# iacopoermacora/Street-sparse-3DGS

Measured on AMD Instinct MI355X. Metric: fwd+bwd Mpix/s at 1080p (1M Gaussians), higher is better.
Workload: dtype f32; 1 GPU; rasterizer fwd+bwd, 1000000 Gaussians, SH degree 3, 1920x1080, do_depth; gaussians=1000000, width=1920, height=1080, sh_degree=3, tiles=8160, fwd_segment=2048, parallelism=chunk-per-gpu x1

## Files before the change

### street-sparse-3dgs_amd/csrc/backward.hip

```cpp
#include <algorithm>
#include <atomic>

#include "gsr_launch.h"

namespace gsr {

#ifndef GSR_RED_SERIAL
#define GSR_RED_SERIAL 32
#endif
constexpr uint32_t kRedSerial = GSR_RED_SERIAL;
#ifndef GSR_REC_BATCH
#define GSR_REC_BATCH 4
#endif
#ifndef GSR_LIVE_UNROLL
#define GSR_LIVE_UNROLL 8
#endif
#ifndef GSR_BIG_BLOCK
#define GSR_BIG_BLOCK 2
#endif
constexpr int kRecBatch = GSR_REC_BATCH;

template <int D, bool kRow = false>
__device__ __forceinline__ void sh_backward(const float *__restrict__ sh, int M, bool vec, const float dir[3],
                                            const float gc[3], float *__restrict__ dsh, float gd[3]) {
// ... 188 lines not shown
            for (int j = 0; j < kBigBlock; j++) {
                q[0] += ra[j].x; q[1] += ra[j].y; q[2] += ra[j].z; q[3] += ra[j].w;
                q[4] += rb[j].x; q[5] += rb[j].y; q[6] += rb[j].z; q[7] += rb[j].w;
                q[8] += rc[j].x; q[9] += rc[j].y;
            }
        }
#pragma unroll
        for (int k = 0; k < 10; k++) {
            const float t = wave_sum(q[k]);
            if (lane == bl) g[k] = t;
        }
    }
    if (!valid) return;
    dmeans2D[3 * i + 0] = g[0];
    dmeans2D[3 * i + 1] = g[1];
    dmeans2D[3 * i + 2] = 0.f;
    dopacity[i] = g[5];
    sc.gsum[2 * (size_t)i] = make_float4(g[2], g[3], g[4], g[9]);
    sc.gsum[2 * (size_t)i + 1] = make_float4(g[6], g[7], g[8], 0.f);
}

constexpr int kShPitch = 13;
__device__ __forceinline__ void st_out(float *p, float v) { __builtin_nontemporal_store(v, p); }
__device__ __forceinline__ void st_out(float4 *p, float4 v) {
    typedef float f4 __attribute__((ext_vector_type(4)));
    __builtin_nontemporal_store(f4{v.x, v.y, v.z, v.w}, reinterpret_cast<f4 *>(p));
}

__device__ __forceinline__ void geom_chain(int i, float3 p, const Mat4 &V, const float *__restrict__ projmatrix, float fx,
                                           float fy, float tanx, float tany, bool has_scales,
                                           const float *__restrict__ scales, const float *__restrict__ rotations,
                                           float mod, const float *__restrict__ cov3D_precomp, const float g[10],
                                           float c3[6], float4 &q, float3 &s_in, float dm[3], float dcov[6],
                                           int raw) {
    if (has_scales) {
        s_in = make_float3(scales[3 * i], scales[3 * i + 1], scales[3 * i + 2]);
        q = reinterpret_cast<const float4 *>(rotations)[i];
        if (raw) {
            s_in = make_float3(act_scale(s_in.x), act_scale(s_in.y), act_scale(s_in.z));
            q = act_rot(q);
        }
        cov3d_from_scale_rot(s_in, mod, q, c3);
    } else {
#pragma unroll
        for (int k = 0; k < 6; k++) c3[k] = cov3D_precomp[6 * i + k];
    }
    const Ewa e = ewa_rows(p, V, fx, fy, tanx, tany);
    const float a = quad_form(e.m0, c3, e.m0) + 0.3f;
    const float b = quad_form(e.m0, c3, e.m1);
    const float c = quad_form(e.m1, c3, e.m1) + 0.3f;
    const float gca = g[2], gcb = g[3], gcc = g[4];
    const float denom = a * c - b * b;
    const float denom2inv = 1.0f / ((denom * denom) + 0.0000001f);
    float dL_da = 0.f, dL_db = 0.f, dL_dc = 0.f;
    if (denom2inv != 0.f) {
        dL_da = denom2inv * (-c * c * gca + 2.f * b * c * gcb + (denom - a * c) * gcc);
        dL_dc = denom2inv * (-a * a * gcc + 2.f * a * b * gcb + (denom - a * c) * gca);
        dL_db = denom2inv * 2.f * (b * c * gca - (denom + 2.f * b * b) * gcb + a * b * gcc);
        const float *m0 = e.m0, *m1 = e.m1;
        dcov[0] = m0[0] * m0[0] * dL_da + m0[0] * m1[0] * dL_db + m1[0] * m1[0] * dL_dc;
        dcov[3] = m0[1] * m0[1] * dL_da + m0[1] * m1[1] * dL_db + m1[1] * m1[1] * dL_dc;
        dcov[5] = m0[2] * m0[2] * dL_da + m0[2] * m1[2] * dL_db + m1[2] * m1[2] * dL_dc;
        dcov[1] = 2.f * m0[0] * m0[1] * dL_da + (m0[0] * m1[1] + m0[1] * m1[0]) * dL_db +
                  2.f * m1[0] * m1[1] * dL_dc;
        dcov[2] = 2.f * m0[0] * m0[2] * dL_da + (m0[0] * m1[2] + m0[2] * m1[0]) * dL_db +
                  2.f * m1[0] * m1[2] * dL_dc;
        dcov[4] = 2.f * m0[2] * m0[1] * dL_da + (m0[1] * m1[2] + m0[2] * m1[1]) * dL_db +
                  2.f * m1[1] * m1[2] * dL_dc;
    }
    float Sm0[3], Sm1[3];
    const float *m0 = e.m0, *m1 = e.m1;
    Sm0[0] = c3[0] * m0[0] + c3[1] * m0[1] + c3[2] * m0[2];
    Sm0[1] = c3[1] * m0[0] + c3[3] * m0[1] + c3[4] * m0[2];
    Sm0[2] = c3[2] * m0[0] + c3[4] * m0[1] + c3[5] * m0[2];
    Sm1[0] = c3[0] * m1[0] + c3[1] * m1[1] + c3[2] * m1[2];
    Sm1[1] = c3[1] * m1[0] + c3[3] * m1[1] + c3[4] * m1[2];
    Sm1[2] = c3[2] * m1[0] + c3[4] * m1[1] + c3[5] * m1[2];
    float dm0[3], dm1[3];
#pragma unroll
    for (int k = 0; k < 3; k++) {
        dm0[k] = 2.f * Sm0[k] * dL_da + Sm1[k] * dL_db;
        dm1[k] = 2.f * Sm1[k] * dL_dc + Sm0[k] * dL_db;
    }
    const float *v = V.m;
    const float dj00 = v[0] * dm0[0] + v[4] * dm0[1] + v[8] * dm0[2];
    const float dj02 = v[2] * dm0[0] + v[6] * dm0[1] + v[10] * dm0[2];
    const float dj11 = v[1] * dm1[0] + v[5] * dm1[1] + v[9] * dm1[2];
    const float dj12 = v[2] * dm1[0] + v[6] * dm1[1] + v[10] * dm1[2];
    const float tz = 1.f / e.t.z, tz2 = tz * tz, tz3 = tz2 * tz;
    const float dtx = e.xmul * -fx * tz2 * dj02;
    const float dty = e.ymul * -fy * tz2 * dj12;
    const float dtz = -fx * tz2 * dj00 - fy * tz2 * dj11 + (2.f * fx * e.t.x) * tz3 * dj02 +
                      (2.f * fy * e.t.y) * tz3 * dj12;
    dm[0] = v[0] * dtx + v[1] * dty + v[2] * dtz;
    dm[1] = v[4] * dtx + v[5] * dty + v[6] * dtz;
    dm[2] = v[8] * dtx + v[9] * dty + v[10] * dtz;

    const Mat4 Pm = load_mat4(projmatrix);
    const float *pr = Pm.m;
    const float4 mh = xf_point44(p, Pm);
    const float mw = 1.0f / (mh.w + 0.0000001f);
    const float mul1 = mh.x * mw * mw, mul2 = mh.y * mw * mw;
    dm[0] += (pr[0] * mw - pr[3] * mul1) * g[0] + (pr[1] * mw - pr[3] * mul2) * g[1];
    dm[1] += (pr[4] * mw - pr[7] * mul1) * g[0] + (pr[5] * mw - pr[7] * mul2) * g[1];
    dm[2] += (pr[8] * mw - pr[11] * mul1) * g[0] + (pr[9] * mw - pr[11] * mul2) * g[1];

    {
        const float3 pv = xf_point43(p, V);
        const float dz = -g[9] / (pv.z * pv.z);
        dm[0] += dz * v[2];
        dm[1] += dz * v[6];
        dm[2] += dz * v[10];
    }
}

__device__ __forceinline__ void scale_rot_chain(float4 q, float3 s_in, float mod, float dscale_mod, const float dcov[6],
                                                float ds[3], float dq[4]) {
    const float r = q.x, x = q.y, y = q.z, z = q.w;
    const float s[3] = {mod * s_in.x, mod * s_in.y, mod * s_in.z};
    const Rot3 R = quat_to_rot(q);
    const float G3[3][3] = {{dcov[0], 0.5f * dcov[1], 0.5f * dcov[2]},
                            {0.5f * dcov[1], dcov[3], 0.5f * dcov[4]},
                            {0.5f * dcov[2], 0.5f * dcov[4], dcov[5]}};
    float dLL[3][3];
#pragma unroll
    for (int rr = 0; rr < 3; rr++)
#pragma unroll
        for (int cc = 0; cc < 3; cc++)
            dLL[rr][cc] = 2.f * (G3[rr][0] * R.m[0][cc] * s[cc] + G3[rr][1] * R.m[1][cc] * s[cc] +
                                 G3[rr][2] * R.m[2][cc] * s[cc]);
#pragma unroll
// ... 280 lines not shown
        st_out(&out.dscales[3 * i + 0], 0.f);
        st_out(&out.dscales[3 * i + 1], 0.f);
        st_out(&out.dscales[3 * i + 2], 0.f);
    }
    if (valid && !live) st_out(&reinterpret_cast<float4 *>(out.drots)[i], z4);
    float4 *dst4 = reinterpret_cast<float4 *>(out.dsh) + row0 * 12;
#pragma unroll
    for (int k = 0; k < 12; k++) {
        const int f = k * kWave + lane, row = f / 12;
        if (row0 + row < P && !((lm >> row) & 1ull)) st_out(&dst4[f], z4);
    }
}

constexpr int kLiveRange = 2048;
constexpr int kLiveBlocksPerCU = 2;

struct LiveArgs {
    int P, D;
    const float *means3D, *shs;
    const uint8_t *clamped;
    const float *scales, *rotations;
    float mod, dscale_mod;
    const float *viewmatrix, *projmatrix, *campos;
    float tanx, tany, fx, fy;
    BwdScratch sc;
    GaussianGrads out;
    int raw, stamped;
    StepAct act;
};

__device__ __forceinline__ void live_row(int i, const Mat4 &V, int D, const float *__restrict__ means3D,
                                         const float *__restrict__ shs, const uint8_t *__restrict__ clamped,
                                         const float *__restrict__ scales, const float *__restrict__ rotations,
                                         float mod, float dscale_mod, const float *__restrict__ projmatrix,
                                         const float *__restrict__ campos_p, float tanx, float tany, float fx, float fy,
                                         const BwdScratch &sc, const GaussianGrads &out, int raw, int stamped,
                                         const StepAct &act) {
    float g[10];
    load_sums(sc, out, i, true, g);
    const float3 p = make_float3(means3D[3 * i], means3D[3 * i + 1], means3D[3 * i + 2]);
    float dm[3] = {0.f, 0.f, 0.f};
    float dcov[6] = {0.f, 0.f, 0.f, 0.f, 0.f, 0.f};
    float c3[6];
    float4 q = make_float4(0.f, 0.f, 0.f, 0.f);
    float3 s_in = make_float3(0.f, 0.f, 0.f);
    geom_chain(i, p, V, projmatrix, fx, fy, tanx, tany, true, scales, rotations, mod, nullptr, g, c3, q,
               s_in, dm, dcov, raw);
    if (stamped) {
        st_out(&out.dmeans2D[3 * i + 0], g[0]);
        st_out(&out.dmeans2D[3 * i + 1], g[1]);
        st_out(&out.dmeans2D[3 * i + 2], out.sparse_rows ? 1.f : 0.f);
        st_out(&out.dopacity[i], g[5]);
    }
    if (sc.atomic) {
        float4 *acc = sc.acc + 4 * (size_t)i;
        const float4 z4 = make_float4(0.f, 0.f, 0.f, 0.f);
#pragma unroll
        for (int k = 0; k < 4; k++) acc[k] = z4;
    }
    float dir[3], dor[3];
    sh_dir(p, make_float3(campos_p[0], campos_p[1], campos_p[2]), dir, dor);
    const uint8_t cl = clamped[i];
    float gc[3];
#pragma unroll
    for (int ch = 0; ch < 3; ch++) gc[ch] = (cl >> ch) & 1 ? 0.f : g[6 + ch];
    float gd[3];
    const float *sh = shs + (size_t)i * 48;
    float *dsh = out.dsh + (size_t)i * 48;
    switch (D) {
        case 0: sh_backward<0>(sh, 16, true, dir, gc, dsh, gd); break;
        case 1: sh_backward<1>(sh, 16, true, dir, gc, dsh, gd); break;
        case 2: sh_backward<2>(sh, 16, true, dir, gc, dsh, gd); break;
        default: sh_backward<3>(sh, 16, true, dir, gc, dsh, gd); break;
    }
    dir_chain(dor, gd, dm);
    st_out(&out.dmeans3D[3 * i + 0], dm[0]);
    st_out(&out.dmeans3D[3 * i + 1], dm[1]);
    st_out(&out.dmeans3D[3 * i + 2], dm[2]);
    float ds[3], dq[4];
    scale_rot_chain(q, s_in, mod, dscale_mod, dcov, ds, dq);
    if (act.on) {
#pragma unroll
        for (int k = 0; k < 3; k++) ds[k] = ds[k] * act_scale(act.s_raw[3 * i + k]);
        const float4 x = act.q_raw[i];
        const float4 gq = make_float4(dq[0], dq[1], dq[2], dq[3]);
        const float nq = sqrtf(x.x * x.x + x.y * x.y + x.z * x.z + x.w * x.w);
        const float d = fmaxf(nq, 1e-12f);
        const float gd =
            -(gq.x * ((x.x / d) / d) + gq.y * ((x.y / d) / d) + gq.z * ((x.z / d) / d) + gq.w * ((x.w / d) / d));
        const float gn = nq >= 1e-12f && nq != 0.f ? gd / nq : 0.f;
        dq[0] = gq.x / d + x.x * gn;
        dq[1] = gq.y / d + x.y * gn;
        dq[2] = gq.z / d + x.z * gn;
        dq[3] = gq.w / d + x.w * gn;
        const float y = act_opacity(act.o_raw[i]);
        const float go = (int64_t)i < act.skybox ? 0.f : g[5] * (1.f - y) * y;
        st_out(&out.dopacity[i], go);
        if (go != 0.f) *act.flag = 1;
        const int r = act.radii[i];
        if (r > 0) {
            const float gx = g[0], gy = g[1];
            const float nn = sqrtf(gx * gx + gy * gy);
            act.maxr[i] = fmaxf(act.maxr[i], (float)r);
            act.accum[i] = fmaxf(nn, act.accum[i]);
            act.denom[i] = act.denom[i] + 1.f;
        }
    }
    st_out(&out.dscales[3 * i + 0], ds[0]);
    st_out(&out.dscales[3 * i + 1], ds[1]);
    st_out(&out.dscales[3 * i + 2], ds[2]);
    st_out(&reinterpret_cast<float4 *>(out.drots)[i], make_float4(dq[0], dq[1], dq[2], dq[3]));
}

__device__ __forceinline__ void range_compact(const LiveArgs a, int64_t base, const uint32_t *__restrict__ stamps,
                                              uint32_t stamp, uint32_t *s_off, uint8_t *s_byte, uint64_t &m,
                                              uint32_t &byte) {
    const int t = threadIdx.x;
    const int P = a.P;
    const int nw = (P + 63) / 64;
    const int wi = (int)(base / 64) + t / 8;
    if (stamps) {
        byte = 0u;
        const int64_t r0 = base + 8 * t;
#pragma unroll
        for (int k = 0; k < 8; k++)
            if (r0 + k < P && stamps[r0 + k] == stamp) byte |= 1u << k;
        s_byte[t] = (uint8_t)byte;
        __syncthreads();
        m = 0ull;
#pragma unroll
        for (int k = 0; k < 8; k++) m |= (uint64_t)s_byte[(t & ~7) + k] << (8 * k);
    } else {
        m = wi < nw ? a.sc.live[wi] : 0ull;
        byte = (uint32_t)(m >> (8 * (t & 7))) & 0xFFu;
    }
    if ((t & 7) == 0) s_off[t / 8] = (uint32_t)__popcll(m);
    __syncthreads();
    if (t == 0) {
// ... 2 lines not shown
            const uint32_t c = s_off[k];
            s_off[k] = run;
            run += c;
        }
        s_off[kLiveRange / 64] = run;
    }
    __syncthreads();
}

__device__ __forceinline__ void nonlive_stats(const LiveArgs a, int64_t base, uint32_t byte) {
    if (!a.act.on) return;
    const int64_t r0 = base + 8 * threadIdx.x;
#pragma unroll
    for (int k = 0; k < 8; k++) {
        const int64_t i = r0 + k;
        if (i >= a.P || ((byte >> k) & 1u)) continue;
        const int r = a.act.radii[i];
        if (r > 0) {
            const float nn = sqrtf(0.f * 0.f + 0.f * 0.f);
            a.act.maxr[i] = fmaxf(a.act.maxr[i], (float)r);
            a.act.accum[i] = fmaxf(nn, a.act.accum[i]);
            a.act.denom[i] = a.act.denom[i] + 1.f;
        }
    }
}

__global__ __launch_bounds__(256) void grad_range_kernel(
    int P, int D, const float *__restrict__ means3D, const float *__restrict__ shs, const uint8_t *__restrict__ clamped,
    const float *__restrict__ scales, const float *__restrict__ rotations, float mod, float dscale_mod,
    const float *__restrict__ viewmatrix, const float *__restrict__ projmatrix, const float *__restrict__ campos_p,
    float tanx, float tany, float fx, float fy, BwdScratch sc, GaussianGrads out, int raw,
    const uint32_t *__restrict__ stamps, uint32_t stamp, StepAct act) {
    GSR_KS(kKsGradRange);
    __shared__ uint16_t s_list[kLiveRange];
    __shared__ uint32_t s_off[kLiveRange / 64 + 1];
    __shared__ uint8_t s_byte[256];
    const int t = threadIdx.x;
    const int64_t base = (int64_t)blockIdx.x * kLiveRange;
    LiveArgs a{};
    a.P = P;
    a.sc = sc;
    a.act = act;
    uint64_t m;
    uint32_t byte;
    range_compact(a, base, stamps, stamp, s_off, s_byte, m, byte);
    {
        uint32_t pos = s_off[t / 8] + (uint32_t)__popcll(m & ((1ull << (8 * (t & 7))) - 1ull));
        for (uint32_t b = byte; b; b &= b - 1u) s_list[pos++] = (uint16_t)(8 * t + __builtin_ctz(b));
    }
    __syncthreads();
    const uint32_t n = s_off[kLiveRange / 64];
    nonlive_stats(a, base, byte);
    const Mat4 V = load_mat4(viewmatrix);
    for (uint32_t e = (uint32_t)t; e < n; e += blockDim.x)
        live_row((int)(base + s_list[e]), V, D, means3D, shs, clamped, scales, rotations, mod, dscale_mod, projmatrix,
                 campos_p, tanx, tany, fx, fy, sc, out, raw, stamps != nullptr, act);
}

__global__ __launch_bounds__(256) void grad_live_list_kernel(LiveArgs a, const uint32_t *__restrict__ stamps,
                                                             uint32_t stamp, uint32_t *__restrict__ ctr) {
    GSR_KS(kKsLiveList);
    __shared__ uint32_t s_off[kLiveRange / 64 + 1];
    __shared__ uint8_t s_byte[256];
    __shared__ uint32_t s_base;
    const int t = threadIdx.x;
    const int64_t base = (int64_t)blockIdx.x * kLiveRange;
    uint64_t m;
    uint32_t byte;
    range_compact(a, base, stamps, stamp, s_off, s_byte, m, byte);
    if (t == 0) {
        const uint32_t n = s_off[kLiveRange / 64];
        s_base = n ? __hip_atomic_fetch_add(ctr, n, __ATOMIC_RELAXED, __HIP_MEMORY_SCOPE_AGENT) : 0u;
    }
    __syncthreads();
    uint32_t pos = s_base + s_off[t / 8] + (uint32_t)__popcll(m & ((1ull << (8 * (t & 7))) - 1ull));
    for (uint32_t b = byte; b; b &= b - 1u) a.sc.list[pos++] = (uint32_t)(base + 8 * t + __builtin_ctz(b));
    nonlive_stats(a, base, byte);
}

__global__ __launch_bounds__(256) void grad_live_kernel(LiveArgs a, uint32_t *__restrict__ ctr) {
    GSR_KS(kKsGradLive);
    const uint32_t n = __hip_atomic_load(ctr, __ATOMIC_RELAXED, __HIP_MEMORY_SCOPE_AGENT);
    const Mat4 V = load_mat4(a.viewmatrix);
    for (uint32_t e = blockIdx.x * blockDim.x + threadIdx.x; e < n; e += gridDim.x * blockDim.x) {
        const int i_ = (int)a.sc.list[e];
        live_row(i_, V, a.D, a.means3D, a.shs, a.clamped, a.scales, a.rotations, a.mod, a.dscale_mod, a.projmatrix, a.campos,
                 a.tanx, a.tany, a.fx, a.fy, a.sc, a.out, a.raw, a.stamped, a.act);
    }
    __syncthreads();
    if (threadIdx.x == 0 &&
        __hip_atomic_fetch_add(&ctr[1], 1u, __ATOMIC_ACQ_REL, __HIP_MEMORY_SCOPE_AGENT) == gridDim.x - 1u) {
        __hip_atomic_store(&ctr[0], 0u, __ATOMIC_RELAXED, __HIP_MEMORY_SCOPE_AGENT);
        __hip_atomic_store(&ctr[1], 0u, __ATOMIC_RELAXED, __HIP_MEMORY_SCOPE_AGENT);
    }
}

#ifndef GSR_BWD_ZERO_PCT
#define GSR_BWD_ZERO_PCT 100
#endif

namespace {
bool split_ok(const GaussianInputs &in, const GaussianGrads &out, const BwdScratch &sc) {
    return sc.live && in.shs && in.M == 16 && !in.cov3D_precomp && in.scales &&
           in.rotations && reinterpret_cast<uintptr_t>(in.shs) % 16 == 0 &&
           reinterpret_cast<uintptr_t>(out.dsh) % 16 == 0;
}
}

bool bwd_zero_rows(const GaussianInputs &in, const GaussianGrads &out, const BwdScratch &sc, uint32_t *gs_stamps,
                   int nblocks, ZeroRows *z) {
    if (in.P == 0 || nblocks <= 0 || !sc.atomic || !gs_stamps || !split_ok(in, out, sc))
        return false;
    const uint64_t P = (uint64_t)in.P;
    float *p[kZeroArrays] = {out.dmeans2D, out.dopacity, out.dsh, out.dmeans3D, out.dscales, out.drots};
    const uint64_t n[kZeroArrays] = {3 * P, P, 48 * P, 3 * P, 3 * P, 4 * P};
    const int na = out.sparse_rows ? 2 : kZeroArrays;
    for (int k = 0; k < na; k++)
        if (!p[k] || (reinterpret_cast<uintptr_t>(p[k]) & 15u)) return false;
    z->c4[0] = 0;
// ... 57 lines not shown
```

### street-sparse-3dgs_amd/csrc/binning.hip

```cpp
#include "gsr_launch.h"

namespace gsr {

namespace {

constexpr uint32_t kNone = 0xFFFFFFFFu;

struct TileRect {
    int x0, y0, x1, y1;
};

__device__ __forceinline__ TileRect unpack_rect(uint2 d) {
    TileRect r;
    r.x0 = (int)(d.x & 0xFFFFu);
    r.y0 = (int)(d.x >> 16);
    r.x1 = (int)(d.y & 0xFFFFu) - 1;
    r.y1 = (int)(d.y >> 16) - 1;
    return r;
}

__device__ __forceinline__ uint2 load_drect(const uint2 *__restrict__ drect, const uint32_t *__restrict__ drect4, int j) {
    return drect4 ? unpack_rect4(drect4[j]) : drect[j];
}

// ... 90 lines not shown
    __syncthreads();
    const int pv = culled ? P - (int)min(*culled, (uint32_t)P) : P;
    const int j0 = chunk * sg.chunk, j1 = min(pv, j0 + sg.chunk);
    const int side = 1 << sg.shift;
    const auto count = [&](const TileRect &r, const SBWalk &c) {
        const int h = min(r.y1, c.sy * side + side - 1) - max(r.y0, c.sy * side) + 1;
        const int w = min(r.x1, c.sx * side + side - 1) - max(r.x0, c.sx * side) + 1;
        atomicAdd(&cg[c.key], 1u);
        atomicAdd(&ci[c.key], (uint32_t)(w * h));
    };
    for (int jb = j0; jb < j1; jb += 1024) {
        const int j = jb + (int)threadIdx.x;
        const TileRect r = j < j1 ? unpack_rect(load_drect(drect, drect4, j)) : TileRect{0, 0, -1, -1};
        const SBFoot f = sb_foot(r, sg.shift);
        const bool small = f.n <= kSmallSB;
        SBWalk c(f, sg.nsbx);
        for (int k = 0; small && k < f.n; k++, c.next()) count(r, c);
        for (uint64_t big = __ballot(!small); big; big &= big - 1) {
            const int b = __ffsll((unsigned long long)big) - 1;
            const SBFoot fb = lane_foot(f, b);
            const TileRect rb = lane_rect(r, b);
            const int dy = 64 / fb.sw, dx = 64 - dy * fb.sw;
            SBWalk cb(fb, sg.nsbx, (int)(threadIdx.x & 63));
            for (int k = threadIdx.x & 63; k < fb.n; k += 64, cb.skip(dy, dx)) count(rb, cb);
        }
    }
    __syncthreads();
    for (int s = threadIdx.x; s < sg.nsb; s += 1024) {
        cnt_g[(size_t)s * sg.ccols + cnt_col(sg, chunk)] = cg[s];
        cnt_i[(size_t)s * sg.ccols + cnt_col(sg, chunk)] = ci[s];
    }
}

template <int NT>
__device__ __forceinline__ uint32_t block_exclusive_scan(uint32_t v, uint32_t *wsum, uint32_t &total) {
    constexpr int kW = NT / 64;
    const int lane = threadIdx.x & 63, w = threadIdx.x >> 6;
    uint32_t incl = v;
#pragma unroll
    for (int o = 1; o < 64; o <<= 1) {
        const uint32_t t = (uint32_t)__shfl_up((int)incl, o, 64);
        if (lane >= o) incl += t;
    }
    __syncthreads();
    if (lane == 63) wsum[w] = incl;
    __syncthreads();
    uint32_t before = 0;
    total = 0;
#pragma unroll
    for (int k = 0; k < kW; k++) {
        before += k < w ? wsum[k] : 0u;
        total += wsum[k];
    }
    return before + incl - v;
}

#ifndef GSR_SORT_CAP
#define GSR_SORT_CAP 8192
#endif
constexpr int kSBThreads = 1024;
constexpr int kSBWaves = kSBThreads / 64;
constexpr int kSortCap = GSR_SORT_CAP;
constexpr int kSBItems = kSortCap / kSBThreads;
static_assert(kSortCap % kSBThreads == 0 && kSortCap <= 65536, "kSortCap: a multiple of 1024, 16-bit positions");

constexpr int kColThreads = 256;
__global__ __launch_bounds__(kColThreads) void sb_colscan_kernel(SBGrid sg, uint32_t *__restrict__ cnt_g,
                                                                 const uint32_t *__restrict__ cnt_i,
                                                                 uint32_t *__restrict__ base_g,
                                                                 uint32_t *__restrict__ base_i,
                                                                 uint32_t *__restrict__ done, FrameWords fw,
                                                                 uint32_t *__restrict__ tb_flag,
                                                                 uint32_t *__restrict__ tb_items, uint32_t tb_len,
                                                                 uint32_t *__restrict__ host_sblist, int P,
                                                                 const uint32_t *__restrict__ culled) {
    GSR_KS(kKsSbColscan);
    __shared__ uint32_t wsum[kColThreads / 64];
    __shared__ uint32_t s_last, s_tb;
    const int s = blockIdx.x;
    uint32_t *row = cnt_g + (size_t)s * sg.ccols;
    const uint32_t *rowi = cnt_i + (size_t)s * sg.ccols;
    uint32_t carry = 0, isum = 0;
    const int nch = visible_chunks(sg, P, culled);
    for (int b = 0; b < nch; b += kColThreads) {
        const int c = b + (int)threadIdx.x;
        const uint32_t v = c < nch ? row[cnt_col(sg, c)] : 0u;
        isum += c < nch ? rowi[cnt_col(sg, c)] : 0u;
        uint32_t tot;
        const uint32_t ex = block_exclusive_scan<kColThreads>(v, wsum, tot);
        if (c < nch) row[cnt_col(sg, c)] = carry + ex;
        carry += tot;
    }
    uint32_t itot;
    (void)block_exclusive_scan<kColThreads>(isum, wsum, itot);
    if (threadIdx.x == 0) {
        __hip_atomic_store(&base_g[s], carry, __ATOMIC_RELAXED, __HIP_MEMORY_SCOPE_AGENT);
        __hip_atomic_store(&base_i[s], itot, __ATOMIC_RELAXED, __HIP_MEMORY_SCOPE_AGENT);
        asm volatile("s_waitcnt vmcnt(0)" ::: "memory");
        const uint32_t prev = __hip_atomic_fetch_add(done, 1u, __ATOMIC_RELAXED, __HIP_MEMORY_SCOPE_AGENT);
        s_last = prev == gridDim.x - 1u;
    }
    __syncthreads();
    if (!s_last) return;
    const int nsb = sg.nsb;
    if (threadIdx.x == 0) s_tb = 0u;
    __syncthreads();
    uint32_t cg = 0, ci = 0, mg = 0;
    for (int b = 0; b < nsb; b += kColThreads) {
        const int k = b + (int)threadIdx.x;
        const uint32_t vg = k < nsb ? __hip_atomic_load(&base_g[k], __ATOMIC_RELAXED, __HIP_MEMORY_SCOPE_AGENT) : 0u;
        const uint32_t vi = k < nsb ? __hip_atomic_load(&base_i[k], __ATOMIC_RELAXED, __HIP_MEMORY_SCOPE_AGENT) : 0u;
        mg = max(mg, vg);
        if (tb_flag && k < nsb) {
            uint32_t nsl = tb_len && vg > tb_len ? min((vg + tb_len - 1u) / tb_len, kTBMaxSlices) : 0u;
            const uint32_t at = nsl ? atomicAdd(&s_tb, nsl) : 0u;
            const bool fits = nsl && at + nsl <= (uint32_t)kTBMaxItems;
            for (uint32_t j = 0; j < nsl && at + j < (uint32_t)kTBMaxItems; j++)
                tb_items[at + j] = fits ? ((uint32_t)k | j << 12 | nsl << 18) : kTBVoid;
            tb_flag[k] = fits ? 1u : 0u;
        }
        uint32_t tg, ti;
        const uint32_t eg = block_exclusive_scan<kColThreads>(vg, wsum, tg);
        const uint32_t ei = block_exclusive_scan<kColThreads>(vi, wsum, ti);
        if (k < nsb) {
            base_g[k] = cg + eg;
            base_i[k] = ci + ei;
        }
        cg += tg;
        ci += ti;
    }
    if (threadIdx.x == 0) {
        base_g[nsb] = cg;
        base_i[nsb] = ci;
    }
    if (tb_flag) {
        __syncthreads();
        if (threadIdx.x == 0) tb_flag[nsb] = min(s_tb, (uint32_t)kTBMaxItems);
    }
    if (fw.dev_K || host_sblist) {
        mg = wave_max_u32(mg);
        __syncthreads();
        if ((threadIdx.x & 63) == 0) wsum[threadIdx.x >> 6] = mg;
        __syncthreads();
        if (threadIdx.x == 0) {
            for (int k = 1; k < kColThreads / 64; k++) mg = max(mg, wsum[k]);
            if (host_sblist) __hip_atomic_store(host_sblist, mg, __ATOMIC_RELAXED, __HIP_MEMORY_SCOPE_SYSTEM);
        }
    }
    if (fw.dev_K) {
        if (threadIdx.x == 0) {
            *fw.dev_K = mg > (uint32_t)kSortCap ? 0xFFFFFFFFu : ci;
            *fw.dev_maxsb = mg;
            if (fw.host) {
                __hip_atomic_store(&fw.host[kHostMaxSB], mg, __ATOMIC_RELAXED, __HIP_MEMORY_SCOPE_SYSTEM);
                __hip_atomic_store(&fw.host[kHostP1], cg, __ATOMIC_RELAXED, __HIP_MEMORY_SCOPE_SYSTEM);
                __hip_atomic_store(&fw.host[kHostK], ci, __ATOMIC_RELEASE, __HIP_MEMORY_SCOPE_SYSTEM);
            }
        }
    }
}

__device__ __forceinline__ void mask_or(uint64_t *m, uint64_t bit) {
// ... 660 lines not shown
```

### street-sparse-3dgs_amd/csrc/gsr_device.h

```cpp
#pragma once
#include <hip/hip_runtime.h>
#include <stdint.h>

namespace gsr {

constexpr int kTile = 16;
constexpr int kWave = 64;
constexpr int kPixPerLane = kTile * kTile / kWave;

#define GSR_SH_C0 0.28209479177387814f
#define GSR_SH_C1 0.4886025119029199f
#define GSR_SH_C2_0 1.0925484305920792f
#define GSR_SH_C2_1 -1.0925484305920792f
#define GSR_SH_C2_2 0.31539156525252005f
#define GSR_SH_C2_3 -1.0925484305920792f
#define GSR_SH_C2_4 0.5462742152960396f
#define GSR_SH_C3_0 -0.5900435899266435f
#define GSR_SH_C3_1 2.890611442640554f
#define GSR_SH_C3_2 -0.4570457994644658f
#define GSR_SH_C3_3 0.3731763325901154f
#define GSR_SH_C3_4 -0.4570457994644658f
#define GSR_SH_C3_5 1.445305721320277f
#define GSR_SH_C3_6 -0.5900435899266435f

// ... 331 lines not shown
                 GSR_DPP_KEEP("row_half_mirror", "0x5", 3, 8) GSR_DPP_KEEP("row_half_mirror", "0xa", 3, 13)
                 GSR_DPP_KEEP("row_half_mirror", "0x5", 4, 9) GSR_DPP_KEEP("row_half_mirror", "0xa", 4, 14)
                 : "=&v"(c0), "=&v"(c1), "=&v"(c2), "=&v"(c3), "=&v"(c4)
                 : "v"(k0), "v"(k1), "v"(k2), "v"(k3), "v"(k4), "v"(k5), "v"(k6), "v"(k7), "v"(k8), "v"(k9));
    float d0 = b1 ? c3 : c0, d1 = b1 ? c4 : c1, d2 = b1 ? 0.f : c2;
    const float u0 = b1 ? c0 : c3, u1 = b1 ? c1 : c4, u2 = b1 ? c2 : 0.f;
    asm volatile("s_nop 1\n" GSR_DPP_RS("quad_perm:[2,3,0,1]", 0, 3) GSR_DPP_RS("quad_perm:[2,3,0,1]", 1, 4)
                     GSR_DPP_RS("quad_perm:[2,3,0,1]", 2, 5)
                 : "+v"(d0), "+v"(d1), "+v"(d2)
                 : "v"(u0), "v"(u1), "v"(u2));
    float e0 = b0 ? d2 : d0, e1 = b0 ? 0.f : d1;
    const float x0 = b0 ? d0 : d2, x1 = b0 ? d1 : 0.f;
    asm volatile("s_nop 1\n" GSR_DPP_RS("quad_perm:[1,0,3,2]", 0, 2) GSR_DPP_RS("quad_perm:[1,0,3,2]", 1, 3)
                 : "+v"(e0), "+v"(e1)
                 : "v"(x0), "v"(x1));
    const auto r = __builtin_amdgcn_permlane16_swap(__float_as_uint(e0), __float_as_uint(e1), false, false);
    return __uint_as_float(r[0]) + __uint_as_float(r[1]);
}
#undef GSR_DPP_RS
#undef GSR_DPP_KEEP

__device__ __forceinline__ int wave_rs20_slot(int lane) {
    const int b3 = (lane >> 3) & 1, b2 = (lane >> 2) & 1, b1 = (lane >> 1) & 1, b0 = lane & 1, row = (lane >> 4) & 1;
    const int t = row + 2 * b0;
    const int c = t + 3 * b1;
    return (t == 3 || c >= 5) ? -1 : 10 * b3 + 5 * b2 + c;
}

__device__ __forceinline__ int wave_rs10_slot(int lane) {
    const int b3 = (lane >> 3) & 1, b2 = (lane >> 2) & 1, c = lane & 3;
    return (c == 3 || (b2 && c == 2)) ? -1 : 5 * b3 + 3 * b2 + c;
}

template <int kCtrl>
__device__ __forceinline__ uint32_t dpp_u(uint32_t v) {
    return (uint32_t)__builtin_amdgcn_update_dpp(0, (int)v, kCtrl, 0xF, 0xF, false);
}
__device__ __forceinline__ uint32_t wave_max_u32(uint32_t v) {
    v = max(v, dpp_u<0xB1>(v));
    v = max(v, dpp_u<0x4E>(v));
    v = max(v, dpp_u<0x124>(v));
    v = max(v, dpp_u<0x128>(v));
    const auto r16 = __builtin_amdgcn_permlane16_swap(v, v, false, false);
    v = max(r16[0], r16[1]);
    const auto r32 = __builtin_amdgcn_permlane32_swap(v, v, false, false);
    return max(r32[0], r32[1]);
}

constexpr float kLog2e = 1.4426950408889634f;

constexpr float kHalfLog2e = -0.5f * 1.4426950408889634f;
__device__ __forceinline__ float gauss_p2(float adxdx_s, float bdx_s, float c_s, float dy) {
    return fmaf(-bdx_s, dy, fmaf(c_s * dy, dy, adxdx_s));
}

__host__ __device__ inline size_t align_up(size_t x, size_t a) { return (x + a - 1) / a * a; }

struct alignas(16) GRec {
    float x, y, ca, cb;
    float cc, op, ex, ey;
    float r, g, b, invd;
    uint32_t rect0, rectw, dbits;
    float cull_tm;
};
static_assert(sizeof(GRec) == 64, "GRec must be one 64-B line");

#ifndef GSR_SB_CHUNK
#define GSR_SB_CHUNK 1024
#endif
// ... 215 lines not shown
```

Baseline: 3373 Mpix/s.

## Hoist live-row loads, per-wave compaction, DPP wave scan, batched column scans

The live-row backward path now loads the gradient sums, scales, rotations, SH coefficients and activation inputs up front, and passes the projection matrix and camera position as preloaded values. This is meant to issue memory requests early and remove repeated global reads. The range kernel replaces its block-wide compaction (shared offsets plus __syncthreads) with a per-wave DPP inclusive scan, so each wave compacts and processes its own 512 rows with no block barrier. The superblock column scan is rewritten to process several items per thread with fewer barriers, and the last workgroup holds every superblock total in registers. The cost is higher register pressure (48 SH floats per thread) and load imbalance across waves, since each wave now handles only its own rows.

```diff
diff --git a/street-sparse-3dgs_amd/csrc/backward.hip b/street-sparse-3dgs_amd/csrc/backward.hip
--- a/street-sparse-3dgs_amd/csrc/backward.hip
+++ b/street-sparse-3dgs_amd/csrc/backward.hip
@@ -244,10 +244,12 @@
                                            const float *__restrict__ scales, const float *__restrict__ rotations,
                                            float mod, const float *__restrict__ cov3D_precomp, const float g[10],
                                            float c3[6], float4 &q, float3 &s_in, float dm[3], float dcov[6],
-                                           int raw) {
+                                           int raw, bool loaded = false, const Mat4 *proj = nullptr) {
     if (has_scales) {
-        s_in = make_float3(scales[3 * i], scales[3 * i + 1], scales[3 * i + 2]);
-        q = reinterpret_cast<const float4 *>(rotations)[i];
+        if (!loaded) {
+            s_in = make_float3(scales[3 * i], scales[3 * i + 1], scales[3 * i + 2]);
+            q = reinterpret_cast<const float4 *>(rotations)[i];
+        }
         if (raw) {
             s_in = make_float3(act_scale(s_in.x), act_scale(s_in.y), act_scale(s_in.z));
             q = act_rot(q);
@@ -308,7 +310,7 @@
     dm[1] = v[4] * dtx + v[5] * dty + v[6] * dtz;
     dm[2] = v[8] * dtx + v[9] * dty + v[10] * dtz;
 
-    const Mat4 Pm = load_mat4(projmatrix);
+    const Mat4 Pm = proj ? *proj : load_mat4(projmatrix);
     const float *pr = Pm.m;
     const float4 mh = xf_point44(p, Pm);
     const float mw = 1.0f / (mh.w + 0.0000001f);
@@ -655,20 +657,50 @@
 __device__ __forceinline__ void live_row(int i, const Mat4 &V, int D, const float *__restrict__ means3D,
                                          const float *__restrict__ shs, const uint8_t *__restrict__ clamped,
                                          const float *__restrict__ scales, const float *__restrict__ rotations,
-                                         float mod, float dscale_mod, const float *__restrict__ projmatrix,
-                                         const float *__restrict__ campos_p, float tanx, float tany, float fx, float fy,
+                                         float mod, float dscale_mod, const Mat4 &Pm, float3 campos, float tanx,
+                                         float tany, float fx, float fy,
                                          const BwdScratch &sc, const GaussianGrads &out, int raw, int stamped,
                                          const StepAct &act) {
     float g[10];
-    load_sums(sc, out, i, true, g);
+    {
+        const bool at = sc.atomic != 0;
+        const float4 *r4 = at ? sc.acc + 4 * (size_t)i : sc.gsum + 2 * (size_t)i;
+        const float *r2 = at ? reinterpret_cast<const float *>(sc.acc + 4 * (size_t)i + 2) : out.dmeans2D + 3 * (size_t)i;
+        const float *r1 = at ? reinterpret_cast<const float *>(sc.acc + 4 * (size_t)i + 1) + 1 : out.dopacity + i;
+        const float4 v0 = r4[0], v1 = r4[1];
+        const float w0 = r2[0], w1 = r2[1], w2 = r1[0];
+        g[0] = at ? v0.x : w0;   g[1] = at ? v0.y : w1;   g[2] = at ? v0.z : v0.x; g[3] = at ? v0.w : v0.y;
+        g[4] = at ? v1.x : v0.z; g[5] = at ? v1.y : w2;   g[6] = at ? v1.z : v1.x; g[7] = at ? v1.w : v1.y;
+        g[8] = at ? w0 : v1.z;   g[9] = at ? w1 : v0.w;
+    }
     const float3 p = make_float3(means3D[3 * i], means3D[3 * i + 1], means3D[3 * i + 2]);
+    float3 s_in = make_float3(scales[3 * i], scales[3 * i + 1], scales[3 * i + 2]);
+    float4 q = reinterpret_cast<const float4 *>(rotations)[i];
+    const uint8_t cl = clamped[i];
+    float4 sh4[12];
+    {
+        const float4 *s4 = reinterpret_cast<const float4 *>(shs + (size_t)i * 48);
+#pragma unroll
+        for (int k = 0; k < 12; k++) sh4[k] = s4[k];
+    }
+    float a_s[3] = {0.f, 0.f, 0.f}, a_o = 0.f, a_maxr = 0.f, a_accum = 0.f, a_denom = 0.f;
+    float4 a_q = make_float4(0.f, 0.f, 0.f, 0.f);
+    int a_r = 0;
+    if (act.on) {
+#pragma unroll
+        for (int k = 0; k < 3; k++) a_s[k] = act.s_raw[3 * i + k];
+        a_q = act.q_raw[i];
+        a_o = act.o_raw[i];
+        a_r = act.radii[i];
+        a_maxr = act.maxr[i];
+        a_accum = act.accum[i];
+        a_denom = act.denom[i];
+    }
     float dm[3] = {0.f, 0.f, 0.f};
     float dcov[6] = {0.f, 0.f, 0.f, 0.f, 0.f, 0.f};
     float c3[6];
-    float4 q = make_float4(0.f, 0.f, 0.f, 0.f);
-    float3 s_in = make_float3(0.f, 0.f, 0.f);
-    geom_chain(i, p, V, projmatrix, fx, fy, tanx, tany, true, scales, rotations, mod, nullptr, g, c3, q,
-               s_in, dm, dcov, raw);
+    geom_chain(i, p, V, nullptr, fx, fy, tanx, tany, true, scales, rotations, mod, nullptr, g, c3, q,
+               s_in, dm, dcov, raw, true, &Pm);
     if (stamped) {
         st_out(&out.dmeans2D[3 * i + 0], g[0]);
         st_out(&out.dmeans2D[3 * i + 1], g[1]);
@@ -682,13 +714,12 @@
         for (int k = 0; k < 4; k++) acc[k] = z4;
     }
     float dir[3], dor[3];
-    sh_dir(p, make_float3(campos_p[0], campos_p[1], campos_p[2]), dir, dor);
-    const uint8_t cl = clamped[i];
+    sh_dir(p, campos, dir, dor);
     float gc[3];
 #pragma unroll
     for (int ch = 0; ch < 3; ch++) gc[ch] = (cl >> ch) & 1 ? 0.f : g[6 + ch];
     float gd[3];
-    const float *sh = shs + (size_t)i * 48;
+    const float *sh = reinterpret_cast<const float *>(sh4);
     float *dsh = out.dsh + (size_t)i * 48;
     switch (D) {
         case 0: sh_backward<0>(sh, 16, true, dir, gc, dsh, gd); break;
@@ -704,8 +735,8 @@
     scale_rot_chain(q, s_in, mod, dscale_mod, dcov, ds, dq);
     if (act.on) {
 #pragma unroll
-        for (int k = 0; k < 3; k++) ds[k] = ds[k] * act_scale(act.s_raw[3 * i + k]);
-        const float4 x = act.q_raw[i];
+        for (int k = 0; k < 3; k++) ds[k] = ds[k] * act_scale(a_s[k]);
+        const float4 x = a_q;
         const float4 gq = make_float4(dq[0], dq[1], dq[2], dq[3]);
         const float nq = sqrtf(x.x * x.x + x.y * x.y + x.z * x.z + x.w * x.w);
         const float d = fmaxf(nq, 1e-12f);
@@ -716,17 +747,17 @@
         dq[1] = gq.y / d + x.y * gn;
         dq[2] = gq.z / d + x.z * gn;
         dq[3] = gq.w / d + x.w * gn;
-        const float y = act_opacity(act.o_raw[i]);
+        const float y = act_opacity(a_o);
         const float go = (int64_t)i < act.skybox ? 0.f : g[5] * (1.f - y) * y;
         st_out(&out.dopacity[i], go);
         if (go != 0.f) *act.flag = 1;
-        const int r = act.radii[i];
+        const int r = a_r;
         if (r > 0) {
             const float gx = g[0], gy = g[1];
             const float nn = sqrtf(gx * gx + gy * gy);
-            act.maxr[i] = fmaxf(act.maxr[i], (float)r);
-            act.accum[i] = fmaxf(nn, act.accum[i]);
-            act.denom[i] = act.denom[i] + 1.f;
+            act.maxr[i] = fmaxf(a_maxr, (float)r);
+            act.accum[i] = fmaxf(nn, a_accum);
+            act.denom[i] = a_denom + 1.f;
         }
     }
     st_out(&out.dscales[3 * i + 0], ds[0]);
@@ -795,29 +826,51 @@
     float tanx, float tany, float fx, float fy, BwdScratch sc, GaussianGrads out, int raw,
     const uint32_t *__restrict__ stamps, uint32_t stamp, StepAct act) {
     GSR_KS(kKsGradRange);
+    constexpr int kWaveRows = 8 * kWave;
+    static_assert(kLiveRange == 4 * kWaveRows, "256 threads, eight rows per lane");
     __shared__ uint16_t s_list[kLiveRange];
-    __shared__ uint32_t s_off[kLiveRange / 64 + 1];
-    __shared__ uint8_t s_byte[256];
-    const int t = threadIdx.x;
+    const int t = threadIdx.x, lane = t & (kWave - 1);
     const int64_t base = (int64_t)blockIdx.x * kLiveRange;
+    const int64_t wbase = base + (int64_t)(t / kWave) * kWaveRows;
+    const int64_t r0 = base + 8 * t;
+    uint16_t *const list = s_list + (t / kWave) * kWaveRows;
     LiveArgs a{};
     a.P = P;
     a.sc = sc;
     a.act = act;
-    uint64_t m;
-    uint32_t byte;
-    range_compact(a, base, stamps, stamp, s_off, s_byte, m, byte);
+    const Mat4 V = load_mat4(viewmatrix), Pm = load_mat4(projmatrix);
+    const float3 campos = make_float3(campos_p[0], campos_p[1], campos_p[2]);
+    uint32_t byte = 0u;
+    if (stamps) {
+        if (wbase + kWaveRows <= P && reinterpret_cast<uintptr_t>(stamps) % 16 == 0) {
+            const uint4 s0 = reinterpret_cast<const uint4 *>(stamps + r0)[0];
+            const uint4 s1 = reinterpret_cast<const uint4 *>(stamps + r0)[1];
+            byte = (uint32_t)(s0.x == stamp) | (uint32_t)(s0.y == stamp) << 1 | (uint32_t)(s0.z == stamp) << 2 |
+                   (uint32_t)(s0.w == stamp) << 3 | (uint32_t)(s1.x == stamp) << 4 | (uint32_t)(s1.y == stamp) << 5 |
+                   (uint32_t)(s1.z == stamp) << 6 | (uint32_t)(s1.w == stamp) << 7;
+        } else {
+#pragma unroll
+            for (int k = 0; k < 8; k++)
+                if (r0 + k < P && stamps[r0 + k] == stamp) byte |= 1u << k;
+        }
+    } else {
+        const int wi = (int)(base / 64) + t / 8;
+        const uint64_t m = wi < (P + 63) / 64 ? sc.live[wi] : 0ull;
+        byte = (uint32_t)(m >> (8 * (t & 7))) & 0xFFu;
+    }
+    const uint32_t cnt = (uint32_t)__popc(byte);
+    const uint32_t incl = wave_inclusive_sum_u32(cnt);
+    const uint32_t n = (uint32_t)__builtin_amdgcn_readlane((int)incl, kWave - 1);
     {
-        uint32_t pos = s_off[t / 8] + (uint32_t)__popcll(m & ((1ull << (8 * (t & 7))) - 1ull));
-        for (uint32_t b = byte; b; b &= b - 1u) s_list[pos++] = (uint16_t)(8 * t + __builtin_ctz(b));
-    }
-    __syncthreads();
-    const uint32_t n = s_off[kLiveRange / 64];
+        uint32_t pos = incl - cnt;
+        for (uint32_t b = byte; b; b &= b - 1u) list[pos++] = (uint16_t)(8 * lane + __builtin_ctz(b));
+    }
+    __builtin_amdgcn_s_waitcnt(0xc07f);
+    __builtin_amdgcn_wave_barrier();
     nonlive_stats(a, base, byte);
-    const Mat4 V = load_mat4(viewmatrix);
-    for (uint32_t e = (uint32_t)t; e < n; e += blockDim.x)
-        live_row((int)(base + s_list[e]), V, D, means3D, shs, clamped, scales, rotations, mod, dscale_mod, projmatrix,
-                 campos_p, tanx, tany, fx, fy, sc, out, raw, stamps != nullptr, act);
+    for (uint32_t e = (uint32_t)lane; e < n; e += kWave)
+        live_row((int)(wbase + list[e]), V, D, means3D, shs, clamped, scales, rotations, mod, dscale_mod, Pm, campos,
+                 tanx, tany, fx, fy, sc, out, raw, stamps != nullptr, act);
 }
 
 __global__ __launch_bounds__(256) void grad_live_list_kernel(LiveArgs a, const uint32_t *__restrict__ stamps,
@@ -844,10 +897,11 @@
 __global__ __launch_bounds__(256) void grad_live_kernel(LiveArgs a, uint32_t *__restrict__ ctr) {
     GSR_KS(kKsGradLive);
     const uint32_t n = __hip_atomic_load(ctr, __ATOMIC_RELAXED, __HIP_MEMORY_SCOPE_AGENT);
-    const Mat4 V = load_mat4(a.viewmatrix);
+    const Mat4 V = load_mat4(a.viewmatrix), Pm = load_mat4(a.projmatrix);
+    const float3 campos = make_float3(a.campos[0], a.campos[1], a.campos[2]);
     for (uint32_t e = blockIdx.x * blockDim.x + threadIdx.x; e < n; e += gridDim.x * blockDim.x) {
         const int i_ = (int)a.sc.list[e];
-        live_row(i_, V, a.D, a.means3D, a.shs, a.clamped, a.scales, a.rotations, a.mod, a.dscale_mod, a.projmatrix, a.campos,
+        live_row(i_, V, a.D, a.means3D, a.shs, a.clamped, a.scales, a.rotations, a.mod, a.dscale_mod, Pm, campos,
                  a.tanx, a.tany, a.fx, a.fy, a.sc, a.out, a.raw, a.stamped, a.act);
     }
     __syncthreads();
diff --git a/street-sparse-3dgs_amd/csrc/binning.hip b/street-sparse-3dgs_amd/csrc/binning.hip
--- a/street-sparse-3dgs_amd/csrc/binning.hip
+++ b/street-sparse-3dgs_amd/csrc/binning.hip
@@ -146,27 +146,34 @@
     }
 }
 
-template <int NT>
-__device__ __forceinline__ uint32_t block_exclusive_scan(uint32_t v, uint32_t *wsum, uint32_t &total) {
+template <int NT, int R>
+__device__ __forceinline__ void rows_publish(const uint32_t (&v)[R], uint32_t (&incl)[R], uint32_t *sums) {
+    const int lane = threadIdx.x & 63, w = threadIdx.x >> 6;
+#pragma unroll
+    for (int j = 0; j < R; j++) incl[j] = wave_inclusive_sum_u32(v[j]);
+    if (lane == 63)
+#pragma unroll
+        for (int j = 0; j < R; j++) sums[j * (NT / 64) + w] = incl[j];
+}
+template <int NT, int R>
+__device__ __forceinline__ uint32_t rows_collect(const uint32_t (&v)[R], const uint32_t (&incl)[R],
+                                                 const uint32_t *sums, uint32_t (&ex)[R]) {
     constexpr int kW = NT / 64;
-    const int lane = threadIdx.x & 63, w = threadIdx.x >> 6;
-    uint32_t incl = v;
-#pragma unroll
-    for (int o = 1; o < 64; o <<= 1) {
-        const uint32_t t = (uint32_t)__shfl_up((int)incl, o, 64);
-        if (lane >= o) incl += t;
-    }
-    __syncthreads();
-    if (lane == 63) wsum[w] = incl;
-    __syncthreads();
-    uint32_t before = 0;
-    total = 0;
-#pragma unroll
-    for (int k = 0; k < kW; k++) {
-        before += k < w ? wsum[k] : 0u;
-        total += wsum[k];
-    }
-    return before + incl - v;
+    const int w = threadIdx.x >> 6;
+    uint32_t run = 0;
+#pragma unroll
+    for (int j = 0; j < R; j++) {
+        uint32_t before = 0, rowtot = 0;
+#pragma unroll
+        for (int k = 0; k < kW; k++) {
+            const uint32_t sk = sums[j * kW + k];
+            before += k < w ? sk : 0u;
+            rowtot += sk;
+        }
+        ex[j] = run + before + incl[j] - v[j];
+        run += rowtot;
+    }
+    return run;
 }
 
 #ifndef GSR_SORT_CAP
@@ -179,6 +186,10 @@
 static_assert(kSortCap % kSBThreads == 0 && kSortCap <= 65536, "kSortCap: a multiple of 1024, 16-bit positions");
 
 constexpr int kColThreads = 256;
+constexpr int kColItems = 4;
+constexpr int kColTrip = kColThreads * kColItems;
+constexpr int kBaseItems = kMaxSB / kColThreads;
+static_assert(kMaxSB % kColThreads == 0, "the last workgroup holds every superblock's totals in registers");
 __global__ __launch_bounds__(kColThreads) void sb_colscan_kernel(SBGrid sg, uint32_t *__restrict__ cnt_g,
                                                                  const uint32_t *__restrict__ cnt_i,
                                                                  uint32_t *__restrict__ base_g,
@@ -189,24 +200,43 @@
                                                                  uint32_t *__restrict__ host_sblist, int P,
                                                                  const uint32_t *__restrict__ culled) {
     GSR_KS(kKsSbColscan);
-    __shared__ uint32_t wsum[kColThreads / 64];
+    constexpr int kW = kColThreads / 64;
+    __shared__ uint32_t wsum[kBaseItems * kW], wsum_i[kBaseItems * kW];
     __shared__ uint32_t s_last, s_tb;
+    static_assert(kBaseItems >= kColItems, "the column trips use the first rows of the sums");
     const int s = blockIdx.x;
     uint32_t *row = cnt_g + (size_t)s * sg.ccols;
     const uint32_t *rowi = cnt_i + (size_t)s * sg.ccols;
-    uint32_t carry = 0, isum = 0;
+    uint32_t carry = 0, itot = 0;
     const int nch = visible_chunks(sg, P, culled);
-    for (int b = 0; b < nch; b += kColThreads) {
-        const int c = b + (int)threadIdx.x;
-        const uint32_t v = c < nch ? row[cnt_col(sg, c)] : 0u;
-        isum += c < nch ? rowi[cnt_col(sg, c)] : 0u;
-        uint32_t tot;
-        const uint32_t ex = block_exclusive_scan<kColThreads>(v, wsum, tot);
-        if (c < nch) row[cnt_col(sg, c)] = carry + ex;
+    for (int b = 0; b < nch; b += kColTrip) {
+        uint32_t v[kColItems], vi[kColItems], incl[kColItems], ex[kColItems];
+        int at[kColItems];
+#pragma unroll
+        for (int j = 0; j < kColItems; j++) {
+            const int c = b + j * kColThreads + (int)threadIdx.x;
+            at[j] = c < nch ? cnt_col(sg, c) : -1;
+        }
+#pragma unroll
+        for (int j = 0; j < kColItems; j++) v[j] = at[j] >= 0 ? row[at[j]] : 0u;
+#pragma unroll
+        for (int j = 0; j < kColItems; j++) vi[j] = at[j] >= 0 ? rowi[at[j]] : 0u;
+        uint32_t isum = 0;
+#pragma unroll
+        for (int j = 0; j < kColItems; j++) isum += vi[j];
+        rows_publish<kColThreads, kColItems>(v, incl, wsum);
+        isum = wave_inclusive_sum_u32(isum);
+        if ((threadIdx.x & 63) == 63) wsum_i[threadIdx.x >> 6] = isum;
+        __syncthreads();
+        const uint32_t tot = rows_collect<kColThreads, kColItems>(v, incl, wsum, ex);
+#pragma unroll
+        for (int k = 0; k < kW; k++) itot += wsum_i[k];
+#pragma unroll
+        for (int j = 0; j < kColItems; j++)
+            if (at[j] >= 0) row[at[j]] = carry + ex[j];
         carry += tot;
-    }
-    uint32_t itot;
-    (void)block_exclusive_scan<kColThreads>(isum, wsum, itot);
+        if (b + kColTrip < nch) __syncthreads();
+    }
     if (threadIdx.x == 0) {
         __hip_atomic_store(&base_g[s], carry, __ATOMIC_RELAXED, __HIP_MEMORY_SCOPE_AGENT);
         __hip_atomic_store(&base_i[s], itot, __ATOMIC_RELAXED, __HIP_MEMORY_SCOPE_AGENT);
@@ -220,28 +250,44 @@
     if (threadIdx.x == 0) s_tb = 0u;
     __syncthreads();
     uint32_t cg = 0, ci = 0, mg = 0;
-    for (int b = 0; b < nsb; b += kColThreads) {
-        const int k = b + (int)threadIdx.x;
-        const uint32_t vg = k < nsb ? __hip_atomic_load(&base_g[k], __ATOMIC_RELAXED, __HIP_MEMORY_SCOPE_AGENT) : 0u;
-        const uint32_t vi = k < nsb ? __hip_atomic_load(&base_i[k], __ATOMIC_RELAXED, __HIP_MEMORY_SCOPE_AGENT) : 0u;
-        mg = max(mg, vg);
-        if (tb_flag && k < nsb) {
-            uint32_t nsl = tb_len && vg > tb_len ? min((vg + tb_len - 1u) / tb_len, kTBMaxSlices) : 0u;
-            const uint32_t at = nsl ? atomicAdd(&s_tb, nsl) : 0u;
-            const bool fits = nsl && at + nsl <= (uint32_t)kTBMaxItems;
-            for (uint32_t j = 0; j < nsl && at + j < (uint32_t)kTBMaxItems; j++)
-                tb_items[at + j] = fits ? ((uint32_t)k | j << 12 | nsl << 18) : kTBVoid;
-            tb_flag[k] = fits ? 1u : 0u;
-        }
-        uint32_t tg, ti;
-        const uint32_t eg = block_exclusive_scan<kColThreads>(vg, wsum, tg);
-        const uint32_t ei = block_exclusive_scan<kColThreads>(vi, wsum, ti);
-        if (k < nsb) {
-            base_g[k] = cg + eg;
-            base_i[k] = ci + ei;
-        }
-        cg += tg;
-        ci += ti;
+    {
+        uint32_t vg[kBaseItems], vi[kBaseItems], ig[kBaseItems], ii[kBaseItems], eg[kBaseItems], ei[kBaseItems];
+#pragma unroll
+        for (int j = 0; j < kBaseItems; j++) {
+            const int k = j * kColThreads + (int)threadIdx.x;
+            vg[j] = k < nsb ? __hip_atomic_load(&base_g[k], __ATOMIC_RELAXED, __HIP_MEMORY_SCOPE_AGENT) : 0u;
+        }
+#pragma unroll
+        for (int j = 0; j < kBaseItems; j++) {
+            const int k = j * kColThreads + (int)threadIdx.x;
+            vi[j] = k < nsb ? __hip_atomic_load(&base_i[k], __ATOMIC_RELAXED, __HIP_MEMORY_SCOPE_AGENT) : 0u;
+        }
+        rows_publish<kColThreads, kBaseItems>(vg, ig, wsum);
+        rows_publish<kColThreads, kBaseItems>(vi, ii, wsum_i);
+#pragma unroll
+        for (int j = 0; j < kBaseItems; j++) {
+            const int k = j * kColThreads + (int)threadIdx.x;
+            mg = max(mg, vg[j]);
+            if (tb_flag && k < nsb) {
+                uint32_t nsl = tb_len && vg[j] > tb_len ? min((vg[j] + tb_len - 1u) / tb_len, kTBMaxSlices) : 0u;
+                const uint32_t at = nsl ? atomicAdd(&s_tb, nsl) : 0u;
+                const bool fits = nsl && at + nsl <= (uint32_t)kTBMaxItems;
+                for (uint32_t q = 0; q < nsl && at + q < (uint32_t)kTBMaxItems; q++)
+                    tb_items[at + q] = fits ? ((uint32_t)k | q << 12 | nsl << 18) : kTBVoid;
+                tb_flag[k] = fits ? 1u : 0u;
+            }
+        }
+        __syncthreads();
+        cg = rows_collect<kColThreads, kBaseItems>(vg, ig, wsum, eg);
+        ci = rows_collect<kColThreads, kBaseItems>(vi, ii, wsum_i, ei);
+#pragma unroll
+        for (int j = 0; j < kBaseItems; j++) {
+            const int k = j * kColThreads + (int)threadIdx.x;
+            if (k < nsb) {
+                base_g[k] = eg[j];
+                base_i[k] = ei[j];
+            }
+        }
     }
     if (threadIdx.x == 0) {
         base_g[nsb] = cg;
diff --git a/street-sparse-3dgs_amd/csrc/gsr_device.h b/street-sparse-3dgs_amd/csrc/gsr_device.h
--- a/street-sparse-3dgs_amd/csrc/gsr_device.h
+++ b/street-sparse-3dgs_amd/csrc/gsr_device.h
@@ -387,9 +387,18 @@
     return (c == 3 || (b2 && c == 2)) ? -1 : 5 * b3 + 3 * b2 + c;
 }
 
-template <int kCtrl>
+template <int kCtrl, int kRowMask = 0xF>
 __device__ __forceinline__ uint32_t dpp_u(uint32_t v) {
-    return (uint32_t)__builtin_amdgcn_update_dpp(0, (int)v, kCtrl, 0xF, 0xF, false);
+    return (uint32_t)__builtin_amdgcn_update_dpp(0, (int)v, kCtrl, kRowMask, 0xF, false);
+}
+__device__ __forceinline__ uint32_t wave_inclusive_sum_u32(uint32_t v) {
+    v += dpp_u<0x111>(v);
+    v += dpp_u<0x112>(v);
+    v += dpp_u<0x114>(v);
+    v += dpp_u<0x118>(v);
+    v += dpp_u<0x142, 0xA>(v);
+    v += dpp_u<0x143, 0xC>(v);
+    return v;
 }
 __device__ __forceinline__ uint32_t wave_max_u32(uint32_t v) {
     v = max(v, dpp_u<0xB1>(v));
```

After: 3397 Mpix/s, median of 6. Within noise of the previous version (+0.7%).
